# quadram-institute-bioscience/uvaia

Measured on AMD Instinct MI355X. Metric: ref-seqs scored/sec, higher is better.
Workload: dtype u32 bit-planes / int32 counts

## Files before the change

### uvaia_amd/csrc/host_ctx.inc

```

struct uvaia_gpu_ctx;

namespace {

thread_local std::string g_open_error;

int fail(uvaia_gpu_ctx *c, int code, const char *fmt, ...);

#define HIP_TRY(call, on_fail) do { hipError_t e_ = (call); if (e_ != hipSuccess) { const int code_ = e_ == hipErrorOutOfMemory ? UVAIA_GPU_ENOMEM : UVAIA_GPU_EHIP; (void)code_; on_fail; } } while (0)
#define HIPCHK(c, call) HIP_TRY(call, return fail((c), code_, "%s failed: %s (%s:%d)", #call, hipGetErrorString(e_), __FILE__, __LINE__))

template <class T> struct DevBuf {
  T *p = nullptr; size_t cap = 0;
  DevBuf() = default;
  DevBuf(const DevBuf &) = delete; DevBuf &operator=(const DevBuf &) = delete;
  DevBuf(DevBuf &&o) noexcept : p(o.p), cap(o.cap) { o.p = nullptr; o.cap = 0; }
  DevBuf &operator=(DevBuf &&o) noexcept { if (this != &o) { release(); p = o.p; cap = o.cap; o.p = nullptr; o.cap = 0; } return *this; }
  ~DevBuf() { release(); }
  void release() { if (p) hipFree(p); p = nullptr; cap = 0; }
  int reserve(uvaia_gpu_ctx *c, size_t n)
  {
    if (n <= cap) return 0;
    release();
    HIPCHK(c, hipMalloc(&p, n * sizeof(T)));
// ... 6 lines not shown
struct PinnedBuf {
  uint8_t *p = nullptr;
  PinnedBuf() = default;
  PinnedBuf(const PinnedBuf &) = delete; PinnedBuf &operator=(const PinnedBuf &) = delete;
  ~PinnedBuf() { if (p) hipHostFree(p); }
  int alloc(uvaia_gpu_ctx *c, size_t bytes) { HIPCHK(c, hipHostMalloc(&p, bytes, hipHostMallocDefault)); return 0; }
  operator uint8_t *() const { return p; }
};

struct Event {
  hipEvent_t e = nullptr;
  Event() = default;
  Event(const Event &) = delete; Event &operator=(const Event &) = delete;
  Event(Event &&o) noexcept : e(o.e) { o.e = nullptr; }
  Event &operator=(Event &&o) noexcept { if (this != &o) { if (e) hipEventDestroy(e); e = o.e; o.e = nullptr; } return *this; }
  ~Event() { if (e) hipEventDestroy(e); }
  int make(uvaia_gpu_ctx *c, unsigned flags = 0)
  {
    if (e) return 0;
    if (flags) HIPCHK(c, hipEventCreateWithFlags(&e, flags)); else HIPCHK(c, hipEventCreate(&e));
    return 0;
  }
  operator hipEvent_t() const { return e; }
};

struct Stream {
  hipStream_t s = nullptr;
  Stream() = default;
  Stream(const Stream &) = delete; Stream &operator=(const Stream &) = delete;
  ~Stream() { if (s) hipStreamDestroy(s); }
  operator hipStream_t() const { return s; }
};

struct ScanEvt { Event a, b; double bytes = 0; };

struct TileStore {
  DevBuf<uint4> planes;
  DevBuf<int> nonn;
  DevBuf<int> amb;
  DevBuf<int> tot;
  DevBuf<uint4> ev, poly;
  DevBuf<uint32_t> grp;
  DevBuf<int> tote;
};

struct SliceBuf {
  DevBuf<uint32_t> cnt;
  DevBuf<int2> tmin;
  DevBuf<uint32_t> ext;
  DevBuf<uint32_t> rtp;
  DevBuf<uint4> tb8;
  DevBuf<int4> rt;
  int tiles = 0, rb = 0, re = 0; long long tf = 0;
  bool scanned = false, cons_done = false;
  Event scan_done, replay_done;
  bool replay_recorded = false;
};

}

struct uvaia_gpu_ctx {
  int device = 0;
  struct Streams {
    Stream stream;
    Stream scan_streams[3];
    unsigned scan_rr = 0;
    int scan_nstreams = 1;
    int scan_nstreams_forced = 0;
    struct DeriveChunk { long long t0, t1; Event done; };
    Stream derive_streams[3];
    int derive_nstreams = 3; bool derive_forced = false;
    std::vector<DeriveChunk> derive_chunks;
    Event derive_fence[4];
    size_t derive_pending = 0;
    bool planes_busy[4] = {}; hipEvent_t planes_ev[4] = {};
    Stream rep_stream; Event rep_ev[2];
    Event order_ev[16]; unsigned order_rr = 0;
    Event mark_ev[8][3]; bool mark_set[8][3] = {};
  } st;
  SliceBuf slice[NBUF];
  bool use_ext = false;
  size_t subslice = 25088;
  bool subslice_forced = false;
  int first_slice_pct = 70;
  int nq = 0, nq_pad = 0, nchar = 0, W = 0, W4 = 0, P = 4, NQ = 6, acgt = 0, k = 2, qt = 16, n_idx_c = 0, n_idx_m = 0;
  size_t trim = 0;
  size_t max_pool = 0, pool_pad = 0;
  int scan_variant = 2;
  int derive_waves = 0;
  int act_q0 = 0, act_q1 = 0;
  bool serial = false;
  int replay_lq = -1;
  int replay_prio = 1;
  int replay_half = 32;
  int replay_cus = 0;
  int scan_R = 2;
  int scan_NW = 8;
  bool fullscan = false;
  struct QueryTables {
    DevBuf<uint32_t> d_qp;
    DevBuf<uint32_t> d_qp2;
    DevBuf<uint32_t> d_cls;
    DevBuf<uint32_t> d_qpl;
    DevBuf<uint32_t> d_stream;
    DevBuf<uint32_t> d_sdir;
    int NP = 0, NP4 = 0;
    int NR = 0, NR4 = 0, rare_max = -1;
    DevBuf<uint32_t> d_rmask;
    DevBuf<int> d_split;
    DevBuf<uint32_t> d_qrare;
    int need_e_groups = 0, need_v_groups = 0, need_g_groups = 0, need_r_groups = 0;
    DevBuf<int> d_amb_q;
    struct { const void *p; size_t n; } qtab[10] = {};
    DevBuf<uint32_t> d_cp;
    DevBuf<uint32_t> d_cpm;
    DevBuf<uint32_t> d_qpoly;
    DevBuf<uint32_t> d_pmask;
  } tab;
  struct SearchState {
    DevBuf<int> d_heap, d_n, d_T, d_snap, d_err;
    DevBuf<int4> d_cnt;
    DevBuf<int4> d_rt, d_tr;
    DevBuf<uint8_t> d_entered;
    size_t entered_clean = 0;
  } state;
  struct Ball {
    DevBuf<int> d_mindist, d_list, d_cdist, d_n;
    DevBuf<uint4> d_tiles; unsigned long long asked = 0;
    bool fused = true; DevBuf<uint4> d_ga;
    Event ev[4]; double ms[3] = {0., 0., 0.};
    DevBuf<int> d_idx_cols; int n_idx = 0, NG4 = 0;
    std::vector<int> idx_cols; DevBuf<uint32_t> d_masks; int NH4 = 0;
    DevBuf<uint32_t> d_qg;
    DevBuf<unsigned long long> d_key;
    DevBuf<uint4> d_pk; int pk_n = 0;
    DevBuf<uint8_t> d_rows;
    DevBuf<int> d_row_idx;
  } ball;
  struct Rows {
    DevBuf<int> d_sel, d_cnt; DevBuf<unsigned long long> d_off; DevBuf<uint2> d_exc;
    std::vector<int> host; std::vector<uint2> exc_host;
    uint32_t run_cut = 0xFFFFFFu;
    std::vector<Event> evs; double ms[3] = {0., 0., 0.};
  } rows;
  struct Window {
    Stream copy_stream;
    struct StageSlot { DevBuf<uint4> planes; DevBuf<int> nonn, side; int n_tiles = 0; Event copied, read; bool read_recorded = false; };
    StageSlot stage[2];
    DevBuf<int> d_sel;
    DevBuf<uint4> d_four; int n = 0;
    Event ev[5]; double ms[3] = {0., 0., 0.};
    struct Compact { DevBuf<uint4> base; DevBuf<unsigned long long> hidx, lidx; DevBuf<uint32_t> heads, lits; Event ev[3]; bool timed = false; double ms[2] = {0., 0.}; } compact;
  } win;
  struct Shard {
    int rank = 0, world = 1; long long pt = 0;
    const uint4 *peer_db[64] = {}; const int *peer_amb[64] = {};
    void *ipc_opened[64][2] = {};
  } shard;
  TileStore batch;
  DevBuf<uint8_t> d_stage;
  PinnedBuf h_stage;
  Event stage_free[2]; bool stage_busy[2] = {};
  size_t pitch = 0;
  TileStore db;
  size_t db_cap = 0, db_n = 0, db_local_tiles = 0;
  struct { const TileStore *store = nullptr; long long tile_first = 0; int n_tiles = 0, n = 0, rbegin = 0, ppad = 0; const int4 *rt = nullptr; } last;
  struct Stats {
// ... 47 lines not shown
```

### uvaia_amd/csrc/host_launch.inc

```

namespace {

template <class F>
static void parallel_for(int n, F f)
{
  const unsigned nt = std::min<unsigned>(std::max(1u, std::thread::hardware_concurrency()), 64u);
  if (n < 32 || nt < 2) { for (int i = 0; i < n; i++) f(i); return; }
  std::atomic<int> next(0);
  std::vector<std::thread> th;
  for (unsigned t = 0; t < nt; t++) th.emplace_back([&]() { for (;;) { const int a = next.fetch_add(4); if (a >= n) break; for (int i = a; i < std::min(n, a + 4); i++) f(i); } });
  for (auto &x : th) x.join();
}

__global__ void mask_query_planes_kernel(const uint32_t *__restrict__ qp, const uint32_t *__restrict__ pmask, uint32_t *__restrict__ out, size_t n_words_total, int words_per_row, int nq_planes)
{
  const size_t i = (size_t)blockIdx.x * blockDim.x + threadIdx.x;
  if (i >= n_words_total) return;
  const int w = (int)((i / (size_t)nq_planes) % (size_t)words_per_row);
  out[i] = qp[i] & pmask[w];
}

int ensure_qpoly(uvaia_gpu_ctx *c)
{
  if (c->tab.d_qpoly) return 0;
// ... 183 lines not shown
  if (!stream) stream = c->st.stream;
  const bool cons = c->n_idx_c > 0;
  if (cons && !rt) return fail(c, UVAIA_GPU_ESTATE, "no buffer for the consensus pre-score");
  const uint4 *tiles = s.planes; const int *tot_tile0 = s.tot + tile_first * 64;
  const long long ptile_first = tile_first;
  auto consensus_rt = [&]() {
    if (!cons) return;
    if (c->acgt) hipLaunchKernelGGL((consensus_rt_kernel<true>), dim3((n_tiles + 3) / 4), dim3(256), 0, stream, tiles, ptile_first, n_tiles, c->W4, c->tab.d_cp, rt);
    else         hipLaunchKernelGGL((consensus_rt_kernel<false>), dim3((n_tiles + 3) / 4), dim3(256), 0, stream, tiles, ptile_first, n_tiles, c->W4, c->tab.d_cp, rt);
  };
  const int qt2 = c->qt != 8 ? 16 : c->nq <= 1 ? 1 : c->nq <= 2 ? 2 : c->nq <= 4 ? 4 : 8;
  const int n_qtiles = (c->nq + qt2 - 1) / qt2;
  dim3 grid(scan_grid_size(n_qtiles, n_tiles)), block(256);
  ScanEvt ev_{};
  if (c->stats.profile) {
    { int rc_ = take_scan_events(c, ev_); if (rc_) return rc_; }
    HIPCHK(c, hipEventRecord(ev_.a, stream));
  }
  const uint32_t *qp = c->acgt ? c->tab.d_qp : c->tab.d_qp2;
  if (c->scan_variant == 2) {
    planes_touch(c, stream);
    const int *tote = s.tote + tile_first * 64;
    constexpr int QS = 64;
    if (c->act_q0 % QS) return fail(c, UVAIA_GPU_ESTATE, "the scan works on super-tiles of %d queries: active queries start at a multiple of that", QS);
    const int st_first = c->act_q0 / QS, n_st = (c->act_q1 + QS - 1) / QS - st_first;
    const int R = c->scan_R;
    dim3 grid3(scan_grid_size(n_st, (n_tiles + R - 1) / R));
#define SCAN3_LAUNCH(NWW, A, RR) hipLaunchKernelGGL((scan3_kernel<NWW, A, RR>), grid3, dim3(64 * NWW), 0, stream, s.ev, s.poly, tile_first, n_tiles, c->W4, c->tab.NP4, c->tab.NP4 + c->tab.NR4, c->tab.d_qpl, c->tab.d_stream, c->tab.d_sdir, s.grp, tote, tot_tile0, out, ppad, n_st, tmin, r_lo, r_hi, st_first)
#define SCAN3_NW(A, RR) { if (c->scan_NW == 8) SCAN3_LAUNCH(8, A, RR); else SCAN3_LAUNCH(4, A, RR); }
    if (R == 4)      { if (c->acgt) SCAN3_LAUNCH(8, true, 4); else SCAN3_LAUNCH(8, false, 4); }
    else if (R == 2) { if (c->acgt) SCAN3_NW(true, 2) else SCAN3_NW(false, 2) }
    else             { if (c->acgt) SCAN3_NW(true, 1) else SCAN3_NW(false, 1) }
#undef SCAN3_NW
#undef SCAN3_LAUNCH
    HIPCHK(c, hipGetLastError());
    if (c->stats.profile) { HIPCHK(c, hipEventRecord(ev_.b, stream)); ev_.bytes = bytes; c->stats.evts.push_back(std::move(ev_)); }
    consensus_rt();
    HIPCHK(c, hipGetLastError());
    if (tb8 && !c->acgt) {
      hipLaunchKernelGGL(tile_bounds_kernel, dim3((unsigned)n_tiles), dim3(256), 0, stream, out, ppad, n_tiles, c->nq, r_lo, r_hi, tb8, cons ? rt : (const int4 *)nullptr, rtp);
      HIPCHK(c, hipGetLastError());
      if (ext) { int rc_ = launch_pair_extras(c, s, ptile_first, n_tiles, ext, ppad, stream); if (rc_) return rc_; }
    }
    return 0;
  }
  const int *amb0 = s.amb;
#define LAUNCH(K, QT, CN) hipLaunchKernelGGL((K<QT, CN>), grid, block, 0, stream, tiles, tile_first, n_tiles, c->W4, qp, out, ppad, n_qtiles, tot_tile0, tmin, r_lo, r_hi, c->tab.d_cp, rt)
#define LAUNCHX(K, QT, CN) hipLaunchKernelGGL((K<QT, CN>), grid, block, 0, stream, tiles, tile_first, n_tiles, c->W4, qp, out, ppad, n_qtiles, tot_tile0, tmin, r_lo, r_hi, c->tab.d_cp, rt, ext, rtp, tb8, amb0, c->tab.d_qp, c->tab.d_amb_q, c->nq)
#define LAUNCH_QT(L, K, CN) switch (qt2) { case 1: L(K, 1, CN); break; case 2: L(K, 2, CN); break; case 4: L(K, 4, CN); break; case 8: L(K, 8, CN); break; default: L(K, 16, CN); }
  if (c->acgt) { if (cons) { LAUNCH_QT(LAUNCH, scan2_acgt_kernel, true) } else { LAUNCH_QT(LAUNCH, scan2_acgt_kernel, false) } }
  else         { if (cons) { LAUNCH_QT(LAUNCHX, scan2_iupac_kernel, true) } else { LAUNCH_QT(LAUNCHX, scan2_iupac_kernel, false) } }
#undef LAUNCH_QT
#undef LAUNCHX
#undef LAUNCH
  HIPCHK(c, hipGetLastError());
  if (c->stats.profile) { HIPCHK(c, hipEventRecord(ev_.b, stream)); ev_.bytes = bytes; c->stats.evts.push_back(std::move(ev_)); }
  return 0;
}

size_t replay3_lds_bytes(const uvaia_gpu_ctx *c)
{ return (size_t)(c->k + 1) * HEAP_ENTRY * sizeof(int) + 128 + (size_t)16 * 1024 + (size_t)2 * c->replay_half * (c->n_idx_c > 0 ? 4 : 3) * 256; }
int ensure_cnt4(uvaia_gpu_ctx *c, size_t elems) { return c->state.d_cnt.reserve(c, elems); }

int collect_events(uvaia_gpu_ctx *c)
{
  for (auto &e : c->stats.evts) {
    HIPCHK(c, hipEventSynchronize(e.b));
    float ms = 0; HIPCHK(c, hipEventElapsedTime(&ms, e.a, e.b));
    c->stats.scan_ms += ms; c->stats.scan_bytes += e.bytes; c->stats.scan_launches++;
    c->stats.ev_pool.push_back(std::move(e.a)); c->stats.ev_pool.push_back(std::move(e.b));
  }
  c->stats.evts.clear();
  return 0;
}

struct ReplayLaunch {
  hipStream_t stream; int q0, q1;
  const uint32_t *cnt, *ext; int ppad; const int4 *rt; const uint32_t *rtp; const int2 *tmin; const uint4 *tb8;
  const uint4 *planes; long long tile_first; const int *nonn, *amb; uint8_t *entered;
  int rb, re; long long ord_base;
  const uint32_t *qpl; const uint4 *poly; int nr4; const uint32_t *qrare;
  int prefetch;
};
int launch_replay(uvaia_gpu_ctx *c, const ReplayLaunch &L)
{
  const dim3 grid(L.q1 - L.q0), block(64);
  const size_t lds = (size_t)(c->k + 1) * HEAP_ENTRY * sizeof(int);
  c->state.entered_clean = 0;
  if (L.poly) planes_touch(c, L.stream);
  if (c->fullscan) {
#define REPLAY(A) hipLaunchKernelGGL((replay_kernel<A>), grid, block, lds, L.stream, c->state.d_cnt, L.ppad, c->state.d_rt, c->state.d_tr, L.nonn, L.rb, L.re, L.ord_base, c->state.d_heap, c->state.d_n, c->state.d_T, c->state.d_snap, L.entered, c->k)
    if (c->acgt) REPLAY(true); else REPLAY(false);
#undef REPLAY
  } else if (L.ext) {
#define REPLAY3(B, H) hipLaunchKernelGGL((replay3_kernel<B, H>), grid, block, replay3_lds_bytes(c), L.stream, L.cnt, L.ext, L.ppad, L.rt, L.rtp, c->tab.d_cp, L.nonn, L.amb, L.rb, L.re, L.ord_base, \
                                         c->state.d_heap, c->state.d_n, c->state.d_T, c->state.d_snap, L.entered, c->k, L.planes, L.tile_first, c->W4, c->tab.d_qp, c->tab.d_amb_q, c->stats.d_stats, L.q0, L.tb8, c->replay_prio)
#define REPLAY3_HALF(B) { if (c->replay_half == 32) REPLAY3(B, 32); else if (c->replay_half == 16) REPLAY3(B, 16); else REPLAY3(B, 8); }
    if (c->n_idx_c > 0) REPLAY3_HALF(true) else REPLAY3_HALF(false)
#undef REPLAY3_HALF
#undef REPLAY3
  } else {
    const int lq_words = (c->replay_lq && !c->acgt && lds + (size_t)c->W4 * 4 * 6 * 4 + 128 <= 64 * 1024) ? c->W4 * 4 * 6 : 0;
#define REPLAY2(A, B, PF_) hipLaunchKernelGGL((replay2_kernel<A, B, PF_>), grid, block, lds + (size_t)lq_words * 4 + 128, L.stream, L.cnt, L.ppad, L.rt, c->tab.d_cp, L.nonn, L.amb, L.rb, L.re, L.ord_base, \
                                              c->state.d_heap, c->state.d_n, c->state.d_T, c->state.d_snap, L.entered, c->k, L.planes, L.tile_first, c->W4, c->tab.d_qp, c->tab.d_amb_q, c->stats.d_stats, L.q0, L.tmin, L.qpl, lq_words, c->replay_prio, \
                                              L.poly, c->tab.NP4 + c->tab.NR4, c->tab.NP4, L.nr4, L.qrare)
#define REPLAY2_PF(A, B) { if (L.prefetch == 1) REPLAY2(A, B, 1); else if (L.prefetch == 2) REPLAY2(A, B, 2); else REPLAY2(A, B, 3); }
    if (c->acgt) { if (c->n_idx_c > 0) REPLAY2_PF(true, true) else REPLAY2_PF(true, false) }
    else         { if (c->n_idx_c > 0) REPLAY2_PF(false, true) else REPLAY2_PF(false, false) }
#undef REPLAY2_PF
#undef REPLAY2
  }
  HIPCHK(c, hipGetLastError());
  return 0;
}

int run_batch(uvaia_gpu_ctx *c, const TileStore &s, long long tile_first, int n_tiles, int r_begin, int r_end,
              long long ord_base)
{
  if (r_end <= r_begin) return 0;
  const int ppad = n_tiles * 64;
  const SliceBuf &b = c->slice[0];
  hipLaunchKernelGGL(snapshot_kernel, dim3(1), dim3(256), 0, c->st.stream, c->state.d_T, c->nq, c->state.d_snap);
  if (c->n_idx_c > 0 && c->fullscan) {
    if (c->acgt) hipLaunchKernelGGL((consensus_kernel<true>), dim3((n_tiles + 3) / 4), dim3(256), 0, c->st.stream, s.planes, tile_first, n_tiles, c->W4, c->tab.d_cp, c->state.d_snap, c->state.d_rt, c->state.d_tr);
    else         hipLaunchKernelGGL((consensus_kernel<false>), dim3((n_tiles + 3) / 4), dim3(256), 0, c->st.stream, s.planes, tile_first, n_tiles, c->W4, c->tab.d_cp, c->state.d_snap, c->state.d_rt, c->state.d_tr);
  }
  HIPCHK(c, hipGetLastError());
  const double bytes = (double)(r_end - r_begin) * (double)c->W4 * 16.0 * c->P + (double)c->nq * (double)c->W4 * 16.0 * c->P;
  uint32_t *ext = c->use_ext ? b.ext : nullptr;
  int rc = 0;
  if (c->fullscan) {
    rc = ensure_cnt4(c, (size_t)c->nq_pad * c->pool_pad); if (rc) return rc;
    rc = launch_scan(c, s, tile_first, n_tiles, c->tab.d_qp, c->nq, c->state.d_cnt, ppad, bytes);
  } else rc = launch_scan2(c, s, tile_first, n_tiles, b.cnt, ppad, bytes, nullptr, b.tmin, r_begin, r_end, b.rt, ext, b.rtp, b.tb8);
  if (rc) return rc;
  rc = launch_replay(c, {c->st.stream, 0, c->nq, b.cnt, ext, ppad, b.rt, b.rtp, b.tmin, b.tb8,
                             s.planes, tile_first, s.nonn + tile_first * 64, s.amb + tile_first * 64 * AMB_ROW, c->state.d_entered + tile_first * 64, r_begin, r_end, ord_base,
                             c->scan_variant == 2 ? c->tab.d_qpl : nullptr, s.poly, c->tab.NR4, c->tab.d_qrare, 3});
  if (rc) return rc;
  c->last = {&s, tile_first, n_tiles, r_end - r_begin, r_begin, ppad, c->fullscan ? c->state.d_rt : b.rt};
  return 0;
}

int derive_rows(uvaia_gpu_ctx *c, const TileStore &s, long long slot0, int n_ref, hipStream_t st = nullptr, bool v_in_place = false)
{
  if (!st) st = c->st.stream;
  if (c->fullscan || c->scan_variant != 2 || n_ref <= 0 || !c->tab.d_split) return 0;
  if (st == c->st.stream) planes_touch(c, st);
  const long long a = slot0 / 64, t1 = (slot0 + n_ref - 1) / 64;
  const int nblk = (int)(t1 - a + 1);
  const int waves = c->derive_waves ? c->derive_waves : 4;
#define DERIVE_ALL_W(A, V, N) hipLaunchKernelGGL((derive_all_kernel<A, V, N>), dim3(nblk), dim3(64 * N), 0, st, s.planes, a, a, c->W4, c->tab.d_cls, c->tab.d_rmask, c->tab.d_split + derive_split_offset(N), c->tab.NP4, c->tab.NR4, s.ev, s.tote, s.grp, s.poly)
#define DERIVE_ALL(A, V) { if (waves == 8) DERIVE_ALL_W(A, V, 8); else if (waves == 16) DERIVE_ALL_W(A, V, 16); else DERIVE_ALL_W(A, V, 4); }
  if (c->acgt) { if (v_in_place) DERIVE_ALL(true, false) else DERIVE_ALL(true, true) }
  else         { if (v_in_place) DERIVE_ALL(false, false) else DERIVE_ALL(false, true) }
#undef DERIVE_ALL
#undef DERIVE_ALL_W
  HIPCHK(c, hipGetLastError());
  return 0;
}

int sync_scan_streams(uvaia_gpu_ctx *c) { for (hipStream_t st : c->st.scan_streams) if (st) HIPCHK(c, hipStreamSynchronize(st)); planes_idle(c, false, true); return 0; }
int sync_derive_streams(uvaia_gpu_ctx *c) { for (hipStream_t st : c->st.derive_streams) if (st) HIPCHK(c, hipStreamSynchronize(st)); return 0; }

int slice_reserve(uvaia_gpu_ctx *c, SliceBuf &b, size_t need, size_t ppad)
{
  need = std::max(need, b.cnt.cap);
  if (need <= b.cnt.cap && b.tmin) return 0;
  if (int rc = sync_scan_streams(c)) return rc;
  HIPCHK(c, hipStreamSynchronize(c->st.stream));
  const size_t cap = std::max(need, (size_t)c->nq_pad * c->pool_pad), refs = std::max(cap / (size_t)c->nq_pad, ppad) + 64;
  if (int rc = b.cnt.reserve(c, cap)) return rc;
  if (int rc = b.tmin.reserve(c, cap / 64)) return rc;
  if (c->use_ext) {
    if (int rc = b.ext.reserve(c, cap)) return rc;
    if (int rc = b.tb8.reserve(c, cap / 64)) return rc;
    if (int rc = b.rtp.reserve(c, refs)) return rc;
  }
  return b.rt.reserve(c, refs);
}

static int settle_derive(uvaia_gpu_ctx *c)
{
  if (c->st.derive_pending) { if (int rc = sync_derive_streams(c)) return rc; c->st.derive_pending = 0; }
  return 0;
}


int db_refuse_full(uvaia_gpu_ctx *c) { return fail(c, UVAIA_GPU_ESTATE, "database capacity %zu exceeded: call uvaia_gpu_db_reserve first", c->db_cap); }

int db_make_room(uvaia_gpu_ctx *c, size_t n)
// ... 86 lines not shown
```

### uvaia_amd/csrc/host_resident.inc

```

extern "C" {

int uvaia_gpu_db_reserve(uvaia_gpu_ctx *c, size_t cap)
{
  if (!c) return UVAIA_GPU_EINVAL;
  if (cap <= c->db_cap) return 0;
  if (c->db_n) return fail(c, UVAIA_GPU_ESTATE, "reserve the database before appending to it");
  const size_t tiles = (cap + 63) / 64 + 1;
  const size_t dtiles = derived_tiles(c, tiles) + (c->shard.world > 1 ? 1 : 0);
  if (int rc = store_alloc(c, c->db, dtiles)) return rc;
  c->db_local_tiles = dtiles;
  c->shard.peer_db[c->shard.rank] = c->db.planes; c->shard.peer_amb[c->shard.rank] = c->db.amb;
  c->db_cap = tiles * 64 - 64;
  c->state.entered_clean = 0;
  if (int rc = c->state.d_entered.reserve(c, tiles * 64)) return rc;
  HIPCHK(c, hipMemset(c->state.d_entered, 0, c->state.d_entered.cap));
  return 0;
}

static int db_append_common(uvaia_gpu_ctx *c, const char *const *seq, const char *rows, size_t pitch, const int *non_n, int n_ref)
{
  if (!c) return UVAIA_GPU_EINVAL;
  if (n_ref < 0) return fail(c, UVAIA_GPU_EINVAL, "negative count");
  if (n_ref == 0) return 0;
// ... 74 lines not shown

int uvaia_gpu_db_derived_export(uvaia_gpu_ctx *c, size_t n_tiles, void *e, uint32_t *grp, void *poly, int *tot)
{
  if (!c || !e || !grp || !poly || !tot) return UVAIA_GPU_EINVAL;
  if (c->fullscan || c->scan_variant != 2 || !c->db.ev) return fail(c, UVAIA_GPU_ESTATE, "only the column-compressed scan keeps planes derived for the query set");
  if (c->shard.world > 1) return fail(c, UVAIA_GPU_ESTATE, "a context of a reference shard numbers its derived tiles by piece: read them from a plain context");
  if (n_tiles * 64 > ((c->db_n + 63) / 64) * 64) return fail(c, UVAIA_GPU_EINVAL, "tiles 0..%zu lie outside the database", n_tiles);
  if (!n_tiles) return 0;
  { int rc = settle_derive(c); if (rc) return rc; }
  HIPCHK(c, hipStreamSynchronize(c->st.stream));
  const size_t W4 = (size_t)c->W4, NG = (size_t)(c->tab.NP4 + c->tab.NR4);
  HIPCHK(c, hipMemcpy2D(e, 1024, c->db.ev, 2048, 1024, n_tiles * W4, hipMemcpyDeviceToHost));
  HIPCHK(c, hipMemcpy(grp, c->db.grp, n_tiles * W4 * 64 * sizeof(uint32_t), hipMemcpyDeviceToHost));
  if (NG) HIPCHK(c, hipMemcpy(poly, c->db.poly, n_tiles * NG * 3 * 64 * sizeof(uint4), hipMemcpyDeviceToHost));
  HIPCHK(c, hipMemcpy(tot, c->db.tote, n_tiles * 64 * sizeof(int), hipMemcpyDeviceToHost));
  return 0;
}

int uvaia_gpu_db_append_packed(uvaia_gpu_ctx *c, const void *planes, const int *non_n, const int *side_rows, int n_ref)
{
  if (!c) return UVAIA_GPU_EINVAL;
  if (n_ref < 0) return fail(c, UVAIA_GPU_EINVAL, "negative count");
  if (n_ref == 0) return 0;
  if (!planes || !non_n || (!c->acgt && !side_rows)) return fail(c, UVAIA_GPU_EINVAL, "NULL packed arrays");
  if (c->db_n % 64) return fail(c, UVAIA_GPU_ESTATE, "packed tiles can only follow a whole number of tiles (database holds %zu references)", c->db_n);
  if (int rc = db_make_room(c, (size_t)n_ref)) return rc;
  const size_t tb = uvaia_gpu_db_tile_bytes(c), n_tiles_all = ((size_t)n_ref + 63) / 64;
  const long long t0g = (long long)(c->db_n / 64);
  int rc = for_owned_tiles(c, t0g, t0g + (long long)n_tiles_all, [&](long long gt, long long t0, long long nt) -> int {
    const size_t n_tiles = (size_t)nt, off = (size_t)(gt - t0g);
    const char *pl = reinterpret_cast<const char *>(planes) + off * tb;
    if (!c->acgt) {
      HIPCHK(c, hipMemcpyAsync(reinterpret_cast<char *>(c->db.planes.p) + (size_t)t0 * tb, pl, n_tiles * tb, hipMemcpyHostToDevice, c->st.stream));
      if (int rc = db_import_tiles(c, nullptr, t0, n_tiles)) return rc;
      HIPCHK(c, hipMemcpyAsync(c->db.amb + (size_t)t0 * 64 * AMB_ROW, side_rows + off * 64 * AMB_ROW, n_tiles * 64 * AMB_ROW * sizeof(int), hipMemcpyHostToDevice, c->st.stream));
    } else {
      const size_t chunk = 64;
      DevBuf<uint4> d_tmp;
      if (int rc = d_tmp.reserve(c, chunk * tb / sizeof(uint4))) return rc;
      for (size_t a = 0; a < n_tiles; a += chunk) {
        const size_t m = std::min(chunk, n_tiles - a);
        HIPCHK(c, hipMemcpyAsync(d_tmp, pl + a * tb, m * tb, hipMemcpyHostToDevice, c->st.stream));
        if (int rc = db_import_tiles(c, d_tmp, t0 + (long long)a, m)) return rc;
        HIPCHK(c, hipStreamSynchronize(c->st.stream));
      }
    }
    HIPCHK(c, hipMemcpyAsync(c->db.nonn + (size_t)t0 * 64, non_n + off * 64, n_tiles * 64 * sizeof(int), hipMemcpyHostToDevice, c->st.stream));
    if (int rc = db_sanitise_import(c, (size_t)t0 * 64, n_tiles * 64)) return rc;
    return derive_rows(c, c->db, t0 * 64, (int)(n_tiles * 64));
  });
  if (rc) return rc;
  HIPCHK(c, hipStreamSynchronize(c->st.stream));
  db_commit(c, c->db_n + (size_t)n_ref, 0);
  return 0;
}

struct SubSlice { size_t first, n; bool pool_start; };
#ifndef HEAD_TAIL_NQT
#define HEAD_TAIL_NQT 17
#endif
static std::vector<SubSlice> plan_subslices(const uvaia_gpu_ctx *c, size_t first, size_t n, size_t pool)
{
  std::vector<SubSlice> subs;
  const int nqt = (c->act_q1 + 15) / 16 - c->act_q0 / 16;
  if (c->n_idx_c == 0) pool = std::max<size_t>(n, 1);
  size_t sub = c->subslice;
  if (nqt <= 32) sub /= 2;
  if (nqt < 63) sub = std::min(pool, (sub * 63 / (size_t)std::max(nqt, 1) + 63) / 64 * 64);
  if (nqt < 4) sub = std::min(pool, std::max<size_t>(65536, ((pool + 3) / 4 + 63) / 64 * 64));
  if (c->subslice_forced) sub = std::min(pool, c->subslice);
  for (size_t a = first; a < first + n; a += pool) {
    const size_t pe = std::min(first + n, a + pool);
    if (nqt < HEAD_TAIL_NQT && !c->subslice_forced && pe - a >= 8 * 65536) {
      const size_t head = 65536, tail = 65536, pre = (nqt < 4 && pe - a >= 12 * 65536) ? 131072 : 0, mid = pe - a - head - tail - pre, nm = std::max<size_t>(1, (mid + sub / 2) / sub);
      const size_t each = ((mid + nm - 1) / nm + 63) / 64 * 64;
      subs.push_back({a, head, true});
      for (size_t x = a + head; x < pe - tail - pre; x += each) subs.push_back({x, std::min(each, pe - tail - pre - x), false});
      if (pre) subs.push_back({pe - tail - pre, pre, false});
      subs.push_back({pe - tail, tail, false});
      continue;
    }
    const size_t len = pe - a, ns = std::max<size_t>(1, (len + sub / 2) / sub);
    const size_t each = ((len + ns - 1) / ns + 63) / 64 * 64;
    if (c->first_slice_pct > 0 && c->first_slice_pct < 100 && ns >= 3 && !c->subslice_forced) {
      const size_t first_n = std::max<size_t>(64, each * (size_t)c->first_slice_pct / 100 / 64 * 64), rest = len - first_n;
      const size_t each2 = ((rest + (ns - 1) - 1) / (ns - 1) + 63) / 64 * 64;
      subs.push_back({a, first_n, true});
      for (size_t x = a + first_n; x < pe; x += each2) subs.push_back({x, std::min(each2, pe - x), false});
      continue;
    }
    for (size_t x = a; x < pe; x += each) subs.push_back({x, std::min(each, pe - x), x == a});
  }
  return subs;
}

int uvaia_gpu_db_rederive(uvaia_gpu_ctx *c)
{
  if (!c) return UVAIA_GPU_EINVAL;
  if (!c->db.planes || !c->db_n || c->fullscan || c->scan_variant != 2) return 0;
  HIPCHK(c, hipSetDevice(c->device));
  std::vector<SubSlice> plan;
  if (c->shard.world == 1) plan = plan_subslices(c, 0, c->db_n, c->max_pool);
  else {
    const size_t piece = (size_t)c->shard.pt * 64;
    for (size_t a = (size_t)c->shard.rank * piece; a < c->db_n; a += piece * (size_t)c->shard.world) plan.push_back({a, std::min(piece, c->db_n - a), false});
  }
  const int n_derive_streams = (c->st.derive_forced || plan.size() <= 3) ? c->st.derive_nstreams : 1;
  {
    hipStream_t busy[4] = {c->st.stream, c->st.scan_streams[0], c->st.scan_streams[1], c->st.scan_streams[2]};
    for (int i = 0; i < 4; i++) {
      if (!busy[i] || !c->st.planes_busy[i]) continue;
      hipEvent_t e = c->st.planes_ev[i];
      if (!e) {
        if (int rc = c->st.derive_fence[i].make(c, hipEventDisableTiming)) return rc;
        HIPCHK(c, hipEventRecord(c->st.derive_fence[i], busy[i]));
        planes_fenced(c, busy[i], e = c->st.derive_fence[i]);
      }
      for (int j = 0; j < n_derive_streams; j++) HIPCHK(c, hipStreamWaitEvent(c->st.derive_streams[j], e, 0));
    }
  }
  size_t k = 0;
  long long t_done = 0;
  for (const SubSlice &sl : plan) {
    const long long t0 = std::max(t_done, (long long)(sl.first / 64)), t1 = (long long)((sl.first + sl.n + 63) / 64);
    if (t0 >= t1) continue;
    t_done = t1;
    hipStream_t ds = c->st.derive_streams[k % (size_t)n_derive_streams];
    int rc = for_owned_tiles(c, t0, t1, [&](long long, long long lt, long long nt) -> int { return derive_rows(c, c->db, lt * 64, (int)(nt * 64), ds, true); });
    if (rc) return rc;
    if (k == c->st.derive_chunks.size()) {
      c->st.derive_chunks.emplace_back();
      if (int rc = c->st.derive_chunks.back().done.make(c, hipEventDisableTiming)) { c->st.derive_chunks.pop_back(); return rc; }
    }
    c->st.derive_chunks[k].t0 = t0; c->st.derive_chunks[k].t1 = t1;
    HIPCHK(c, hipEventRecord(c->st.derive_chunks[k].done, ds));
    k++;
  }
  c->st.derive_pending = k;
  return 0;
}

static int run_subslices(uvaia_gpu_ctx *c, const std::vector<SubSlice> &subs, int64_t ordinal_of_db0, int snapshot)
{
  const size_t ns = subs.size();
  size_t issued = 0;
  {
    const int nqt = (c->act_q1 + 15) / 16 - c->act_q0 / 16;
    size_t longest = 0;
    for (const SubSlice &sl : subs) longest = std::max(longest, sl.n);
    const size_t waves = ns ? (size_t)nqt * ((longest + 63) / 64) : 0;
    c->st.scan_nstreams = (waves && waves < 16000 && nqt >= 4 && !c->use_ext) ? 3 : 1;
    if (c->st.scan_nstreams_forced) c->st.scan_nstreams = c->st.scan_nstreams_forced;
  }
  for (size_t i = 0; i < ns; i++) {
    const bool serial_ = c->serial;
    while (issued < ns && issued < i + (serial_ ? 1 : NBUF)) {
      int rc = uvaia_gpu_slice_scan(c, subs[issued].first, subs[issued].n, (int)(issued % NBUF));
      if (rc) return rc;
      issued++;
      if (serial_) (void)sync_scan_streams(c);
    }
    int take = subs[i].pool_start ? 1 : 0;
    if (take && snapshot >= 0) { HIPCHK(c, hipMemcpyAsync(c->state.d_snap, &snapshot, sizeof(int), hipMemcpyHostToDevice, c->st.stream)); HIPCHK(c, hipStreamSynchronize(c->st.stream)); take = 0; }
    int rc = uvaia_gpu_slice_replay(c, (int)(i % NBUF), ordinal_of_db0 + (long long)subs[i].first, take);
    if (rc) return rc;
    if (serial_) hipStreamSynchronize(c->st.stream);
  }
  return 0;
// ... 254 lines not shown
```

### uvaia_amd/csrc/kernels_replay.inc

```

template <bool ACGT>
static __device__ __forceinline__ void assemble_scores(const int4 cnt, const int4 rt, const int4 rc, int nn, int S[6], int &mism)
{
  if (ACGT) {
    const int pmm = cnt.x - rt.x, pba = cnt.y - rt.y;
    S[0] = (pba + rc.y) - (pmm + rc.x);
    S[1] = pba + rc.y;
    S[2] = S[0] - (rc.y - rc.x);
    S[3] = nn;
    S[4] = rc.x + (pmm - cnt.z);
    S[5] = cnt.z;
    mism = S[1] - S[0];
  } else {
    const int p0 = cnt.x - rt.x;
    S[0] = p0 + rc.x;
    S[1] = cnt.y - rt.y + rc.y;
    S[2] = cnt.z - rt.z + rc.z;
    S[3] = cnt.w - rt.w + rc.w;
    S[4] = p0;
    S[5] = nn;
    mism = S[3] - S[0];
  }
}

// ... 551 lines not shown
#pragma unroll
          for (int s_ = 0; s_ < PF; s_++) if (pf_idx[s_] == i) pf_idx[s_] = -1;
          const int rl = base_u + i;
          const int cx = __builtin_amdgcn_readlane(cu.x, i), cy = __builtin_amdgcn_readlane(cu.y, i);
          const int4 ai = CONS ? make_int4(__builtin_amdgcn_readlane(a[u].x, i), __builtin_amdgcn_readlane(a[u].y, i), __builtin_amdgcn_readlane(a[u].z, i), __builtin_amdgcn_readlane(a[u].w, i)) : make_int4(0, 0, 0, 0);
          int4 ri = ai;
          const int nni = (CONS || ACGT) ? __builtin_amdgcn_readlane(nn[u], i) : cur.nn;
          const size_t tile_abs = (size_t)tile_first + (size_t)(rl >> 6);
          if (CONS && ((__ballot(cut[u]) >> i) & 1ull)) ri = wave_truncated_consensus<ACGT>(db, tile_abs, rl & 63, W4, cp_cons, snap, lane);
          int Si[6], mi;
          n_demand++;
          if (ACGT) {
            int mp = qpl ? wave_dense_poly_mismatches(polyp, tile_abs, rl & 63, NPT, NP4, qpl + (size_t)q * NP4 * 16, lane) : wave_acgt_poly_mismatches(db, tile_abs, rl & 63, W4, qrow, lane);
            if (qpl && NR4 > 0) mp += wave_rare_mismatches(polyp, tile_abs, rl & 63, NPT, NP4, NR4, qrare + (size_t)q * NR4 * 12, lane);
            assemble_scores<true>(make_int4(cx, cy, mp, 0), ai, ri, nni, Si, mi);
          } else {
            bool dense;
            const int2 d = wave_iupac_finish(cur, db, tile_abs, rl & 63, W4, qw, qlisted, aq_n, lane, dense);
            n_dense += dense;
            assemble_scores<false>(make_int4(cx, cx + d.x, cx + d.x + d.y, cy), ai, ri, nni, Si, mi);
          }
          const bool accept = (mi < T) && (!full || lex_better(Si, W));
          TT_ADD(t2_finish, tfin_);
          if (!accept) { mask &= mask - 1; continue; }
          TT_START(th_);
          {
            const long long ord = ord_base + (rl - r_begin);
            int v = (int)(unsigned)(ord & 0xffffffffll);
            if ((lane & 7) == 7) v = (int)(ord >> 32);
#pragma unroll
            for (int sidx = 0; sidx < 6; sidx++) if ((lane & 7) == sidx) v = Si[sidx];
            if (lane == 0) entered[rl] = 1;
            if (full && use_mc) wave_replace_root_mc(h, n, v, mc, lane, W, Si);
            else if (full) wave_replace_root(h, n, v, lane);
            else {
              if (lane < HEAP_ENTRY) h[(n + 1) * HEAP_ENTRY + lane] = v;
              __syncthreads();
              wave_sift_up(h, n + 1, lane);
            }
          }
          const bool was_full = full;
          if (!full) n++;
          dirty = true; n_admit++;
          __syncthreads();
          full = (n == k);
          if (full) {
            if (!(was_full && use_mc)) {
#pragma unroll
              for (int sidx = 0; sidx < 6; sidx++) W[sidx] = h[HEAP_ENTRY + sidx];
            }
            if (!was_full && use_mc) mc = wave_minchild_init(h, n, lane);
            T = entry_mismatches<ACGT>(W) + 1;
          }
          TT_ADD(t2_heap, th_);
          mask = __ballot(lane > i && may_enter());
        }
#ifdef REPLAY_TIMING
        if (T > T_used) n_trise++;
#endif
        P &= ~(1ull << tsel[u]);
        if (T != T_used) {
          P = needed() & ~((2ull << tsel[u]) - 1ull);
          unsigned long long inflight = 0ull; int last = -1;
#pragma unroll
          for (int v = 0; v < D; v++) if (v > u && tsel[v] >= 0) { inflight |= (1ull << tsel[v]); last = tsel[v]; }
          if (T > T_used && last >= 0 && (P & ~inflight & ((1ull << last) - 1ull)) != 0ull) regroup = true;
          else P |= inflight;
        }
      }
    }
  }
  if (dirty) {
    __syncthreads();
    for (int i = lane; i < (n + 1) * HEAP_ENTRY; i += 64) hg[i] = h[i];
    if (lane == 0) { n_g[q] = n; T_g[q] = T; }
  }
  if (stats && lane == 0) { atomicAdd(&stats[0], (unsigned long long)n_admit); atomicAdd(&stats[1], (unsigned long long)n_demand); atomicAdd(&stats[2], (unsigned long long)n_dense); }
#ifdef REPLAY_TIMING
  if (stats && lane == 0) { atomicAdd(&stats[4], t2_fetch); atomicAdd(&stats[5], t2_finish); atomicAdd(&stats[6], t2_heap); atomicAdd(&stats[7], t2_group); atomicAdd(&stats[8], n_trise); atomicAdd(&stats[9], n_groups);
                            atomicAdd(&stats[10], wall_clock64() - t2_begin); atomicMax(&stats[11], wall_clock64() - t2_begin); }
#endif
#undef TT_START
#undef TT_ADD
}

#pragma clang diagnostic push
#pragma clang diagnostic ignored "-Winline-asm"
static __device__ __forceinline__ void lds_dma_dword(const void *g, uint32_t lds_byte_addr)
{ asm volatile("s_mov_b32 m0, %0\n\ts_nop 0\n\tglobal_load_lds_dword %1, off" ::"s"(__builtin_amdgcn_readfirstlane(lds_byte_addr)), "v"(g) : "memory", "m0"); }
static __device__ __forceinline__ void lds_dma_dwordx4(const void *g, uint32_t lds_byte_addr)
{ asm volatile("s_mov_b32 m0, %0\n\ts_nop 0\n\tglobal_load_lds_dwordx4 %1, off" ::"s"(__builtin_amdgcn_readfirstlane(lds_byte_addr)), "v"(g) : "memory", "m0"); }
#pragma clang diagnostic pop
static __device__ __forceinline__ void replay_wait_staged() { asm volatile("s_waitcnt vmcnt(0)" ::: "memory"); }
__device__ const uint4 g_replay_zero16 = {0u, 0u, 0u, 0u};
typedef __attribute__((address_space(3))) void replay_lds_void;
template <bool CONS, int HALF >
__global__ __launch_bounds__(64) void replay3_kernel(const uint32_t *__restrict__ cnt , const uint32_t *__restrict__ ext, int ppad,
                                                      const int4 *__restrict__ rt, const uint32_t *__restrict__ rtp , const uint32_t *__restrict__ cp_cons,
                                                      const int *__restrict__ nonn, const int *__restrict__ amb,
                                                      int r_begin, int r_end, long long ord_base, int *__restrict__ heap_g, int *__restrict__ n_g, int *__restrict__ T_g,
                                                      const int *__restrict__ snap_ptr, uint8_t *__restrict__ entered, int k, const uint4 *__restrict__ db, long long tile_first, int W4,
                                                      const uint32_t *__restrict__ qfull, const int *__restrict__ amb_q, unsigned long long *__restrict__ stats, int q_first,
                                                      const uint4 *__restrict__ tb8 , int prio_)
{
  extern __shared__ int h[];
  constexpr int NA = CONS ? 4 : 3, NSUB = 64 / HALF;
  constexpr unsigned long long SUB0 = HALF == 32 ? 0xFFFFFFFFull : HALF == 16 ? 0xFFFFull : 0xFFull;
  static_assert(HALF == 32 || HALF == 16 || HALF == 8, "staging buffers of 32, 16 or 8 tiles");
#ifdef REPLAY_TIMING
  const unsigned long long tt_kernel = wall_clock64();
#endif
  if (prio_) __builtin_amdgcn_s_setprio(3);
  const int q = blockIdx.x + q_first, lane = threadIdx.x;
  int *hg = heap_g + (size_t)q * (k + 1) * HEAP_ENTRY;
  int n = min(max(n_g[q], 0), k), T = T_g[q];
  const int snap = *snap_ptr;
  for (int i = lane; i < (n + 1) * HEAP_ENTRY; i += 64) h[i] = hg[i];
  const uint32_t *crow = cnt + (size_t)q * ppad, *xrow = ext + (size_t)q * ppad;
  const uint32_t *qrow = qfull + (size_t)q * W4 * 4 * 6;
  const int aqv = (lane < AMB_STRIDE) ? amb_q[(size_t)q * AMB_STRIDE + lane] : 0;
  const int aq_n = __shfl(aqv, 0);
  const int aq_w = __shfl(aqv, 1 + ((lane < aq_n && lane < AMB_CAP) ? lane : 0));
  uint32_t *qlisted = reinterpret_cast<uint32_t *>(h + (k + 1) * HEAP_ENTRY);
  constexpr int BR = 16;
  uint4 *bring = reinterpret_cast<uint4 *>(qlisted + 32);
  uint32_t *stage = reinterpret_cast<uint32_t *>(bring + BR * 64);
  const uint32_t stage_lds = (uint32_t)(uintptr_t)(replay_lds_void *)stage, bring_lds = (uint32_t)(uintptr_t)(replay_lds_void *)bring;
  if (lane < 32) qlisted[lane] = 0u;
  __syncthreads();
  if (lane < aq_n && aq_n <= AMB_CAP) atomicOr(&qlisted[aq_w >> 5], 1u << (aq_w & 31));
  __syncthreads();
  bool full = (n == k);
  int W[6] = {0, 0, 0, 0, 0, 0};
  const bool use_mc = k <= 127;
  int mc = 0;
  if (full) {
#pragma unroll
    for (int i = 0; i < 6; i++) W[i] = h[HEAP_ENTRY + i];
    if (use_mc) mc = wave_minchild_init(h, n, lane);
  }
  bool dirty = false;
  unsigned n_admit = 0, n_demand = 0, n_dense = 0, n_open = 0;
#ifdef REPLAY_TIMING
  unsigned long long tt_wait = 0, tt_fetch = 0, tt_admit = 0, tt_tile = 0, tt_late = 0, n_late = 0; const unsigned long long tt_begin = tt_kernel, tt_prologue_end = wall_clock64();
#define TT_START(x) const unsigned long long x = wall_clock64()
#define TT_ADD(acc, x) acc += wall_clock64() - x
#else
#define TT_START(x)
#define TT_ADD(acc, x)
#endif
  const uint4 *tmrow = tb8 + (size_t)q * (ppad >> 6);
  const int n_slice_tiles = (r_end + 63) >> 6, n_rounds = (n_slice_tiles + 63) >> 6;
  auto fetch_bounds = [&](int r) {
    if (r >= n_rounds) return;
    const int t = r * 64 + lane;
    const uint4 *src = t < n_slice_tiles ? tmrow + t : &g_replay_zero16;
    lds_dma_dwordx4(src, bring_lds + (uint32_t)(r & (BR - 1)) * 1024u);
  };
  auto fetch_tile = [&](int t, int b) {
    const uint32_t row = stage_lds + (uint32_t)((b * HALF + (t & (HALF - 1))) * NA) * 256u;
    const size_t r = (size_t)t * 64 + lane;
    lds_dma_dword(crow + r, row);
    lds_dma_dword(xrow + r, row + 256u);
    lds_dma_dword(nonn + r, row + 512u);
    if (CONS) lds_dma_dword(rtp + r, row + 768u);
  };
// ... 195 lines not shown
```

Before: 34.81 million.

## Add lean specialized replay kernel and disable uneven first slice for it

Adds a stripped-down replay2 kernel for the common non-ACGT, non-indexed, no-ext, prefetch-2 case. It drops the ext and rare/poly tables and the template branches, and uses fixed prefetch depths of a tile queue and batched count loads, aiming to cut register pressure and per-row overhead. The subslice planner's first-slice percentage now defaults to auto, which disables the smaller first slice when the lean path applies and replay_lq is 0. This is a second maintained copy of the replay logic, so it risks diverging from the general kernel.

```diff
diff --git a/uvaia_amd/csrc/host_ctx.inc b/uvaia_amd/csrc/host_ctx.inc
--- a/uvaia_amd/csrc/host_ctx.inc
+++ b/uvaia_amd/csrc/host_ctx.inc
@@ -112,7 +112,7 @@
   bool use_ext = false;
   size_t subslice = 25088;
   bool subslice_forced = false;
-  int first_slice_pct = 70;
+  int first_slice_pct = -1;
   int nq = 0, nq_pad = 0, nchar = 0, W = 0, W4 = 0, P = 4, NQ = 6, acgt = 0, k = 2, qt = 16, n_idx_c = 0, n_idx_m = 0;
   size_t trim = 0;
   size_t max_pool = 0, pool_pad = 0;
diff --git a/uvaia_amd/csrc/host_launch.inc b/uvaia_amd/csrc/host_launch.inc
--- a/uvaia_amd/csrc/host_launch.inc
+++ b/uvaia_amd/csrc/host_launch.inc
@@ -289,6 +289,7 @@
   const uint32_t *qpl; const uint4 *poly; int nr4; const uint32_t *qrare;
   int prefetch;
 };
+static bool lean_replay_context(const uvaia_gpu_ctx *c) { return !c->fullscan && !c->use_ext && !c->acgt && c->n_idx_c == 0 && c->k <= 127; }
 int launch_replay(uvaia_gpu_ctx *c, const ReplayLaunch &L)
 {
   const dim3 grid(L.q1 - L.q0), block(64);
@@ -312,8 +313,14 @@
                                               c->state.d_heap, c->state.d_n, c->state.d_T, c->state.d_snap, L.entered, c->k, L.planes, L.tile_first, c->W4, c->tab.d_qp, c->tab.d_amb_q, c->stats.d_stats, L.q0, L.tmin, L.qpl, lq_words, c->replay_prio, \
                                               L.poly, c->tab.NP4 + c->tab.NR4, c->tab.NP4, L.nr4, L.qrare)
 #define REPLAY2_PF(A, B) { if (L.prefetch == 1) REPLAY2(A, B, 1); else if (L.prefetch == 2) REPLAY2(A, B, 2); else REPLAY2(A, B, 3); }
-    if (c->acgt) { if (c->n_idx_c > 0) REPLAY2_PF(true, true) else REPLAY2_PF(true, false) }
-    else         { if (c->n_idx_c > 0) REPLAY2_PF(false, true) else REPLAY2_PF(false, false) }
+    bool lean = lean_replay_context(c) && L.prefetch == 2 && lq_words == 0;
+#ifdef REPLAY_TIMING
+    lean = false;
+#endif
+    if (lean) hipLaunchKernelGGL(replay2_lean_kernel, grid, block, lds + 128, L.stream, L.cnt, L.ppad, L.nonn, L.amb, L.rb, L.re, L.ord_base, c->state.d_heap, c->state.d_n, c->state.d_T, L.entered, c->k,
+                                 L.planes, L.tile_first, c->W4, c->tab.d_qp, c->tab.d_amb_q, c->stats.d_stats, L.q0, L.tmin, c->replay_prio);
+    else if (c->acgt) { if (c->n_idx_c > 0) REPLAY2_PF(true, true) else REPLAY2_PF(true, false) }
+    else              { if (c->n_idx_c > 0) REPLAY2_PF(false, true) else REPLAY2_PF(false, false) }
 #undef REPLAY2_PF
 #undef REPLAY2
   }
diff --git a/uvaia_amd/csrc/host_resident.inc b/uvaia_amd/csrc/host_resident.inc
--- a/uvaia_amd/csrc/host_resident.inc
+++ b/uvaia_amd/csrc/host_resident.inc
@@ -180,8 +180,9 @@
     }
     const size_t len = pe - a, ns = std::max<size_t>(1, (len + sub / 2) / sub);
     const size_t each = ((len + ns - 1) / ns + 63) / 64 * 64;
-    if (c->first_slice_pct > 0 && c->first_slice_pct < 100 && ns >= 3 && !c->subslice_forced) {
-      const size_t first_n = std::max<size_t>(64, each * (size_t)c->first_slice_pct / 100 / 64 * 64), rest = len - first_n;
+    const int first_pct = c->first_slice_pct >= 0 ? c->first_slice_pct : ((lean_replay_context(c) && c->replay_lq == 0) ? 0 : 70);
+    if (first_pct > 0 && first_pct < 100 && ns >= 3 && !c->subslice_forced) {
+      const size_t first_n = std::max<size_t>(64, each * (size_t)first_pct / 100 / 64 * 64), rest = len - first_n;
       const size_t each2 = ((rest + (ns - 1) - 1) / (ns - 1) + 63) / 64 * 64;
       subs.push_back({a, first_n, true});
       for (size_t x = a + first_n; x < pe; x += each2) subs.push_back({x, std::min(each2, pe - x), false});
diff --git a/uvaia_amd/csrc/kernels_replay.inc b/uvaia_amd/csrc/kernels_replay.inc
--- a/uvaia_amd/csrc/kernels_replay.inc
+++ b/uvaia_amd/csrc/kernels_replay.inc
@@ -657,6 +657,157 @@
 #endif
 #undef TT_START
 #undef TT_ADD
+}
+
+__global__ __launch_bounds__(64) void replay2_lean_kernel(const uint32_t *__restrict__ cnt , int ppad, const int *__restrict__ nonn, const int *__restrict__ amb,
+                                                           int r_begin, int r_end, long long ord_base, int *__restrict__ heap_g, int *__restrict__ n_g, int *__restrict__ T_g,
+                                                           uint8_t *__restrict__ entered, int k , const uint4 *__restrict__ db, long long tile_first, int W4,
+                                                           const uint32_t *__restrict__ qfull, const int *__restrict__ amb_q, unsigned long long *__restrict__ stats, int q_first,
+                                                           const int2 *__restrict__ tmin, int prio_)
+{
+  extern __shared__ int h[];
+  if (prio_) __builtin_amdgcn_s_setprio(3);
+  const int q = blockIdx.x + q_first, lane = threadIdx.x;
+  int *hg = heap_g + (size_t)q * (k + 1) * HEAP_ENTRY;
+  int n = min(max(n_g[q], 0), k), T = T_g[q];
+  for (int i = lane; i < (n + 1) * HEAP_ENTRY; i += 64) h[i] = hg[i];
+  __syncthreads();
+  bool full = (n == k);
+  int W[6] = {0, 0, 0, 0, 0, 0};
+  int mc = 0;
+  if (full) {
+#pragma unroll
+    for (int i = 0; i < 6; i++) W[i] = __builtin_amdgcn_readfirstlane(h[HEAP_ENTRY + i]);
+    mc = wave_minchild_init(h, n, lane);
+  }
+  const uint32_t *crow = cnt + (size_t)q * ppad;
+  const uint32_t *qw = qfull + (size_t)q * W4 * 4 * 6;
+  const int aqv = (lane < AMB_STRIDE) ? amb_q[(size_t)q * AMB_STRIDE + lane] : 0;
+  const int aq_n = __builtin_amdgcn_readlane(aqv, 0);
+  const int aq_w = __shfl(aqv, 1 + ((lane < aq_n && lane < AMB_CAP) ? lane : 0));
+  uint32_t *qlisted = reinterpret_cast<uint32_t *>(h + (k + 1) * HEAP_ENTRY);
+  if (lane < 32) qlisted[lane] = 0u;
+  __syncthreads();
+  if (lane < aq_n && aq_n <= AMB_CAP) atomicOr(&qlisted[aq_w >> 5], 1u << (aq_w & 31));
+  __syncthreads();
+  bool dirty = false;
+  unsigned n_admit = 0, n_demand = 0, n_dense = 0;
+  const bool use_tmin = tmin != nullptr;
+  const int2 *tmrow = use_tmin ? tmin + (size_t)q * (ppad >> 6) : nullptr;
+  const int n_slice_tiles = (r_end + 63) >> 6;
+  constexpr int D = 8, PD = 4;
+  int2 nbq[PD];
+#pragma unroll
+  for (int i = 0; i < PD; i++) { nbq[i] = make_int2(-1, 0x7fffffff); if (use_tmin && i * 64 + lane < n_slice_tiles) nbq[i] = tmrow[i * 64 + lane]; }
+  for (int tb = 0; tb < n_slice_tiles; tb += 64) {
+    int tm = 0x7fffffff, tk = 0x7fffffff;
+    if (tb + lane < n_slice_tiles) { tm = nbq[0].x; tk = nbq[0].y; }
+#pragma unroll
+    for (int i = 0; i + 1 < PD; i++) nbq[i] = nbq[i + 1];
+    if (use_tmin && tb + PD * 64 + lane < n_slice_tiles) nbq[PD - 1] = tmrow[tb + PD * 64 + lane];
+    auto needed = [&]() -> unsigned long long { return __ballot(tm < T && (!full || tk >= W[0])); };
+    unsigned long long P = needed();
+    while (P) {
+      unsigned long long G;
+      uint32_t craw[D];
+      {
+        unsigned long long rest = P;
+#pragma unroll
+        for (int i = 0; i < D; i++) {
+          craw[i] = 0u;
+          if (rest) {
+            const int r = (tb + (__ffsll((long long)rest) - 1)) * 64 + lane;
+            if (r >= r_begin && r < r_end) craw[i] = crow[r];
+            rest &= rest - 1;
+          }
+        }
+        G = P & ~rest;
+      }
+#pragma unroll 1
+      while (G) {
+        const int t = __ffsll((long long)G) - 1;
+        G &= G - 1;
+        const uint32_t c0 = craw[0];
+#pragma unroll
+        for (int i = 0; i + 1 < D; i++) craw[i] = craw[i + 1];
+        const int K0 = (int)(c0 & 0xFFFFu), K3 = (int)(c0 >> 16);
+        const int T_used = T;
+        const int base_u = (tb + t) * 64;
+        const bool valid = (base_u + lane >= r_begin && base_u + lane < r_end);
+        auto may_enter = [&]() -> bool { return valid && K3 - K0 < T && (!full || K0 >= W[0]); };
+        unsigned long long mask = __ballot(may_enter());
+        auto request = [&](int i_) -> ExtraReq {
+          const int rl_ = base_u + i_;
+          ExtraReq e = wave_iupac_request(db, (size_t)tile_first + (size_t)(rl_ >> 6), rl_ & 63, W4, amb + (size_t)rl_ * AMB_ROW, aq_n, aq_w, lane);
+          e.nn = nonn[rl_];
+          return e;
+        };
+        ExtraReq nxt;
+        int nxt_i = -1;
+        while (mask) {
+          const int i = __ffsll((long long)mask) - 1;
+          const unsigned long long behind = mask & (mask - 1);
+          const int i2 = behind ? (__ffsll((long long)behind) - 1) : -1;
+          ExtraReq cur;
+          if (nxt_i == i) { cur = nxt; nxt_i = -1; }
+          else cur = request(i);
+          if (i2 >= 0 && nxt_i != i2) { nxt = request(i2); nxt_i = i2; }
+          const int rl = base_u + i;
+          const int cx = __builtin_amdgcn_readlane(K0, i), cy = __builtin_amdgcn_readlane(K3, i);
+          const size_t tile_abs = (size_t)tile_first + (size_t)(rl >> 6);
+          int Si[6], mi;
+          n_demand++;
+          bool dense;
+          const int2 d = wave_iupac_finish(cur, db, tile_abs, rl & 63, W4, qw, qlisted, aq_n, lane, dense);
+          n_dense += dense;
+          const int dx = __builtin_amdgcn_readfirstlane(d.x), dy = __builtin_amdgcn_readfirstlane(d.y);
+          assemble_scores<false>(make_int4(cx, cx + dx, cx + dx + dy, cy), make_int4(0, 0, 0, 0), make_int4(0, 0, 0, 0), __builtin_amdgcn_readfirstlane(cur.nn), Si, mi);
+          const bool accept = (mi < T) && (!full || lex_better(Si, W));
+          if (!accept) { mask = behind; continue; }
+          {
+            const long long ord = ord_base + (rl - r_begin);
+            int v = (int)(unsigned)(ord & 0xffffffffll);
+            if ((lane & 7) == 7) v = (int)(ord >> 32);
+#pragma unroll
+            for (int sidx = 0; sidx < 6; sidx++) if ((lane & 7) == sidx) v = Si[sidx];
+            if (lane == 0) entered[rl] = 1;
+            if (full) wave_replace_root_mc(h, n, v, mc, lane, W, Si);
+            else {
+              if (lane < HEAP_ENTRY) h[(n + 1) * HEAP_ENTRY + lane] = v;
+              __syncthreads();
+              wave_sift_up(h, n + 1, lane);
+            }
+          }
+          const bool was_full = full;
+          if (!full) n++;
+          dirty = true; n_admit++;
+          __syncthreads();
+          full = (n == k);
+          if (full) {
+            if (!was_full) {
+#pragma unroll
+              for (int sidx = 0; sidx < 6; sidx++) W[sidx] = __builtin_amdgcn_readfirstlane(h[HEAP_ENTRY + sidx]);
+              mc = wave_minchild_init(h, n, lane);
+            }
+            T = entry_mismatches<false>(W) + 1;
+          }
+          mask = __ballot(lane > i && may_enter());
+        }
+        P &= ~(1ull << t);
+        if (T != T_used) {
+          P = needed() & ~((2ull << t) - 1ull);
+          if (T > T_used && G && (P & ~G & ((1ull << (63 - __clzll((long long)G))) - 1ull)) != 0ull) break;
+          P |= G;
+        }
+      }
+    }
+  }
+  if (dirty) {
+    __syncthreads();
+    for (int i = lane; i < (n + 1) * HEAP_ENTRY; i += 64) hg[i] = h[i];
+    if (lane == 0) { n_g[q] = n; T_g[q] = T; }
+  }
+  if (stats && lane == 0) { atomicAdd(&stats[0], (unsigned long long)n_admit); atomicAdd(&stats[1], (unsigned long long)n_demand); atomicAdd(&stats[2], (unsigned long long)n_dense); }
 }
 
 #pragma clang diagnostic push
```

New measurement: 37.80 million (median of 6 runs). 8.6% higher.
